# LowLevelAI/GLARE

Measured on AMD Instinct MI355X. Metric: enhanced images/sec (400x600), higher is better.
Workload: dtype fp16; 1 GPU; LOL eval15-shaped 400x600 inference, batch=8 per GPU, full encoder->flow->VQ->decoder->AFT (BASELINE configs[1]); batch_per_gpu=8, global_batch=8, input=3x400x600 (reflect-padded to 420x620), parallelism=dp1, streams_per_gpu=2, exchange=none (1 GPU), ranks_seen=1, weights=random, name-seeded (no checkpoints offline)

## Files before the change

### glare_amd/csrc/attn.hip

```cpp
#include <type_traits>

#include "common.h"

namespace {

constexpr int AT_THREADS = 256;
constexpr int HD = 512;
constexpr int BM = 128;
constexpr int BN = 32;
constexpr int KCH = BN * (HD / 8);
constexpr float RESCALE_THR = 8.0f;
constexpr int ATTN_DMA_PER_GROUP = 2;

__device__ __forceinline__ void dma16a(const void* gsrc, void* lds_wave_base) {
  __builtin_amdgcn_global_load_lds((const __attribute__((address_space(1))) void*)gsrc,
                                   (__attribute__((address_space(3))) void*)lds_wave_base, 16, 0, 0);
}

template <int N, typename F>
__device__ __forceinline__ void static_for(F&& f) {
  if constexpr (N > 0) {
    static_for<N - 1>(f);
    f(std::integral_constant<int, N - 1>{});
  }
}

struct AttnParams {
  const a16_t* q;
  const a16_t* k;
  const a16_t* vt;
  a16_t* o;
  int B, N;
  long long Npad;
  int ldq, ldk, ldo;
  int n_qblocks, n_blocks;
  int key_splits;
  float* part_o;
  float* part_ml;
  float* lse;
  a16_t* o_lo;
};

__global__ __launch_bounds__(AT_THREADS, 1) void attn_fwd_kernel(const AttnParams p) {
  extern __shared__ __attribute__((aligned(16))) char smem[];
  u32x4* lK = reinterpret_cast<u32x4*>(smem);
  u32x4* lV = lK + 2 * KCH;

  int bid = blockIdx.x;
  {
    const int n = p.n_blocks, q = n / 8, r = n % 8, xcd = bid % 8, kk = bid / 8;
    bid = (xcd < r ? xcd * (q + 1) : r * (q + 1) + (xcd - r) * q) + kk;
  }
  const int qb = bid % p.n_qblocks, ksplit = (bid / p.n_qblocks) % p.key_splits, b = bid / (p.n_qblocks * p.key_splits);
  const int tid = threadIdx.x, lane = tid & 63;
  const int wave = __builtin_amdgcn_readfirstlane(tid >> 6);
  const int ql = lane & 31, hi = lane >> 5;
  const int qrow = qb * BM + wave * 32 + ql;
  const bool q_ok = qrow < p.N;

  a16x8 qf[HD / 16];
  {
    const a16_t* qp = p.q + ((size_t)b * p.N + (q_ok ? qrow : 0)) * p.ldq + hi * 8;
#pragma unroll
    for (int ks = 0; ks < HD / 16; ++ks) {
      u32x4 v = *reinterpret_cast<const u32x4*>(qp + ks * 16);
      if (!q_ok) v = u32x4{0u, 0u, 0u, 0u};
      qf[ks] = __builtin_bit_cast(a16x8, v);
    }
  }

  f32x16 o[HD / 32];
#pragma unroll
  for (int i = 0; i < HD / 32; ++i)
#pragma unroll
    for (int r = 0; r < 16; ++r) o[i][r] = 0.f;
  float m_run = -1e30f, l_run = 0.f;

  const int n_tiles = (p.N + BN - 1) / BN;
  const int t_begin = (int)((long long)n_tiles * ksplit / p.key_splits), t_end = (int)((long long)n_tiles * (ksplit + 1) / p.key_splits);
  const a16_t* kbase = p.k + (size_t)b * p.N * p.ldk;
  const a16_t* vbase = p.vt + (size_t)b * HD * p.Npad;

  const unsigned v_lane_off = (unsigned)((lane >> 2) * p.Npad + (((lane & 3) ^ ((lane >> 4) & 3)) * 8)) * 2u;
  const __amdgpu_buffer_rsrc_t krsrc = __builtin_amdgcn_make_buffer_rsrc(
      const_cast<a16_t*>(kbase), 0, (int)((((long long)p.N - 1) * p.ldk + HD) * 2), 0x00020000);
  const __amdgpu_buffer_rsrc_t vrsrc =
      __builtin_amdgcn_make_buffer_rsrc(const_cast<a16_t*>(vbase), 0, (int)((long long)HD * p.Npad * 2), 0x00020000);
  const int lane16 = lane * 16;
  auto issue_piece = [&](auto ic, int tile, int buf) {
    constexpr int i = decltype(ic)::value;
    if constexpr (i < BN / 4) {
      const int r = wave + 4 * i;
      __builtin_amdgcn_raw_ptr_buffer_load_lds(krsrc, (__attribute__((address_space(3))) void*)(lK + buf * KCH + r * 64), 16,
                                               lane16 ^ ((r & 15) * 16), (tile * BN + r) * p.ldk * 2, 0, 0);
    } else {
      constexpr int j = i - BN / 4;
      __builtin_amdgcn_raw_ptr_buffer_load_lds(vrsrc, (__attribute__((address_space(3))) void*)(lV + buf * KCH + (wave + 4 * j) * 64), 16,
                                               v_lane_off, (int)(((long long)(wave + 4 * j) * 16 * p.Npad + (long long)tile * BN) * 2), 0, 0);
    }
  };
  auto issue = [&](int tile, int buf) { static_for<16>([&](auto ic) { issue_piece(ic, tile, buf); }); };

  const int krow = (ql & 0x13) | ((ql & 4) << 1) | ((ql & 8) >> 1);
  const int kswz = krow & 15;

  int kofs[8], vofs[2];
#pragma unroll
  for (int bb = 0; bb < 8; ++bb) kofs[bb] = (krow * 64 + ((2 * bb + hi) ^ kswz)) * 16;
#pragma unroll
  for (int ks = 0; ks < 2; ++ks) vofs[ks] = 2 * KCH * 16 + (ql * 4 + ((2 * ks + hi) ^ ((ql >> 2) & 3))) * 16;

  auto tile_body = [&](auto bufc, int tile) {
    constexpr int BUF = decltype(bufc)::value;
    asm volatile("s_waitcnt vmcnt(0)" ::: "memory");
    __syncthreads();
    const int nxt = min(tile + 1, t_end - 1);
    const char* kb = smem + BUF * KCH * 16;
    const char* vb = smem + BUF * KCH * 16;
    a16x8 fr[3][4];
    auto ldk = [&](auto gc, a16x8(&f)[4]) {
      constexpr int g = decltype(gc)::value;
#pragma unroll
      for (int e = 0; e < 4; ++e) {
        const int ks = 4 * g + e;
        f[e] = *reinterpret_cast<const a16x8*>(kb + kofs[ks & 7] + (ks >> 3) * 256);
      }
    };
    auto ldv = [&](auto gc, a16x8(&f)[4]) {
      constexpr int g = decltype(gc)::value;
#pragma unroll
      for (int e = 0; e < 4; ++e) f[e] = *reinterpret_cast<const a16x8*>(vb + vofs[e & 1] + (2 * g + (e >> 1)) * 2048);
    };

    f32x16 s;
#pragma unroll
    for (int r = 0; r < 16; ++r) s[r] = 0.f;
    ldk(std::integral_constant<int, 0>{}, fr[0]);
    ldk(std::integral_constant<int, 1>{}, fr[1]);
    static_for<8>([&](auto gc) {
      constexpr int g = decltype(gc)::value;
      if constexpr (g + 2 < 8) ldk(std::integral_constant<int, g + 2>{}, fr[(g + 2) % 3]);
      else ldv(std::integral_constant<int, g + 2 - 8>{}, fr[(g + 2) % 3]);
      static_for<ATTN_DMA_PER_GROUP>([&](auto kc) {
        constexpr int piece = g * ATTN_DMA_PER_GROUP + decltype(kc)::value;
        if constexpr (piece < 16) issue_piece(std::integral_constant<int, piece>{}, nxt, BUF ^ 1);
      });
#pragma unroll
      for (int e = 0; e < 4; ++e) s = mfma_a16_32x32x16(fr[g % 3][e], qf[4 * g + e], s, 0, 0, 0);
      __builtin_amdgcn_sched_barrier(0);
    });
    if (tile == n_tiles - 1) {
#pragma unroll
      for (int r = 0; r < 16; ++r) {
        const int kv = tile * BN + 16 * (r >> 3) + 8 * hi + (r & 7);
        if (kv >= p.N) s[r] = -__builtin_inff();
      }
    }
    float mx = s[0];
#pragma unroll
    for (int r = 1; r < 16; ++r) mx = fmaxf(mx, s[r]);
    {
      const auto sw = __builtin_amdgcn_permlane32_swap(__float_as_uint(mx), __float_as_uint(mx), false, false);
      mx = fmaxf(mx, __uint_as_float(hi ? sw[0] : sw[1]));
    }
    if (__any(mx > m_run + RESCALE_THR)) {
      const float m_new = fmaxf(m_run, mx);
      const float alpha = __builtin_amdgcn_exp2f(m_run - m_new);
      l_run *= alpha;
#pragma unroll
      for (int i = 0; i < HD / 32; ++i)
#pragma unroll
        for (int r = 0; r < 16; ++r) {
          float x = o[i][r], tmp;
          asm volatile("v_accvgpr_read_b32 %1, %0\n\tv_mul_f32 %1, %1, %2\n\tv_accvgpr_write_b32 %0, %1"
                       : "+a"(x), "=&v"(tmp)
                       : "v"(alpha));
          o[i][r] = x;
        }
      m_run = m_new;
    }
    float psum = 0.f;
    a16x8 pf[2];
#pragma unroll
    for (int h = 0; h < 2; ++h) {
      u32x4 w;
#pragma unroll
      for (int e = 0; e < 4; ++e) {
        const float p0 = __builtin_amdgcn_exp2f(s[8 * h + 2 * e] - m_run);
        const float p1 = __builtin_amdgcn_exp2f(s[8 * h + 2 * e + 1] - m_run);
        psum += p0 + p1;
        w[e] = pack_a2(p0, p1);
      }
      pf[h] = __builtin_bit_cast(a16x8, w);
    }
    l_run += psum;
    __builtin_amdgcn_sched_barrier(0);
    static_for<8>([&](auto gc) {
      constexpr int g = decltype(gc)::value;
      if constexpr (g + 2 < 8) ldv(std::integral_constant<int, g + 2>{}, fr[(8 + g + 2) % 3]);
      static_for<ATTN_DMA_PER_GROUP>([&](auto kc) {
        constexpr int piece = (8 + g) * ATTN_DMA_PER_GROUP + decltype(kc)::value;
        if constexpr (piece < 16) issue_piece(std::integral_constant<int, piece>{}, nxt, BUF ^ 1);
      });
#pragma unroll
      for (int e = 0; e < 4; ++e)
        o[2 * g + (e >> 1)] = mfma_a16_32x32x16(fr[(8 + g) % 3][e], pf[e & 1], o[2 * g + (e >> 1)], 0, 0, 0);
      __builtin_amdgcn_sched_barrier(0);
    });
  };

  issue(t_begin, 0);
  for (int tile = t_begin; tile < t_end; tile += 2) {
    tile_body(std::integral_constant<int, 0>{}, tile);
    if (tile + 1 < t_end) tile_body(std::integral_constant<int, 1>{}, tile + 1);
  }


  const float l_tot = l_run + __shfl_xor(l_run, 32, 64);
  if (p.key_splits > 1) {
    if (q_ok) {
      const size_t row = ((size_t)b * p.key_splits + ksplit) * p.N + qrow;
      float* po = p.part_o + row * HD;
#pragma unroll
      for (int dt = 0; dt < HD / 32; ++dt)
#pragma unroll
        for (int rq = 0; rq < 4; ++rq) {
          const int d = dt * 32 + 8 * rq + 4 * hi;
          *reinterpret_cast<f32x4*>(po + d) = f32x4{o[dt][4 * rq], o[dt][4 * rq + 1], o[dt][4 * rq + 2], o[dt][4 * rq + 3]};
        }
      if (hi == 0) { p.part_ml[row * 2] = m_run; p.part_ml[row * 2 + 1] = l_tot; }
    }
    return;
  }
  const float inv = 1.0f / l_tot;
  if (p.lse && q_ok && hi == 0) p.lse[(size_t)b * p.N + qrow] = m_run + __builtin_amdgcn_logf(l_tot);
  if (q_ok) {
    a16_t* op = p.o + ((size_t)b * p.N + qrow) * p.ldo;
#pragma unroll
    for (int dt = 0; dt < HD / 32; ++dt)
#pragma unroll
      for (int rq = 0; rq < 4; ++rq) {
        const int d = dt * 32 + 8 * rq + 4 * hi;
        u32x2 w = {pack_a2(o[dt][4 * rq] * inv, o[dt][4 * rq + 1] * inv),
                   pack_a2(o[dt][4 * rq + 2] * inv, o[dt][4 * rq + 3] * inv)};
        *reinterpret_cast<u32x2*>(op + d) = w;
      }
  }
}

typedef __attribute__((ext_vector_type(4))) short s16x4;


__device__ __forceinline__ int kv_swz(int key) { return ((key & 3) << 2) | ((key >> 2) & 3); }

template <int OFF>
__device__ __forceinline__ void tr_read_b64(u32x2& dst, int addr) {
  asm volatile("ds_read_b64_tr_b16 %0, %1 offset:%2" : "=v"(dst) : "v"(addr), "i"(OFF));
}
template <int N>
__device__ __forceinline__ void lgkm_wait8(u32x2 (&f)[8]) {
  asm volatile("s_waitcnt lgkmcnt(%8)"
               : "+v"(f[0]), "+v"(f[1]), "+v"(f[2]), "+v"(f[3]), "+v"(f[4]), "+v"(f[5]), "+v"(f[6]), "+v"(f[7])
               : "i"(N));
}

template <bool PAIR>
__global__ __launch_bounds__(AT_THREADS, 1) void attn_kv_fwd_kernel(const AttnParams p) {
  extern __shared__ __attribute__((aligned(16))) char smem[];
  u32x4* lKV = reinterpret_cast<u32x4*>(smem);

  int bid = blockIdx.x;
  {
    const int n = p.n_blocks, q = n / 8, r = n % 8, xcd = bid % 8, kk = bid / 8;
    bid = (xcd < r ? xcd * (q + 1) : r * (q + 1) + (xcd - r) * q) + kk;
  }
  const int qb = bid % p.n_qblocks, ksplit = (bid / p.n_qblocks) % p.key_splits, b = bid / (p.n_qblocks * p.key_splits);
  const int tid = threadIdx.x, lane = tid & 63;
  const int wave = __builtin_amdgcn_readfirstlane(tid >> 6);
  const int ql = lane & 31, hi = lane >> 5;
  const int qrow = qb * BM + wave * 32 + ql;
  const bool q_ok = qrow < p.N;

  a16x8 qf[HD / 16];
  {
    const a16_t* qp = p.q + ((size_t)b * p.N + (q_ok ? qrow : 0)) * p.ldq + hi * 8;
#pragma unroll
    for (int ks = 0; ks < HD / 16; ++ks) {
      u32x4 v = *reinterpret_cast<const u32x4*>(qp + ks * 16);
      if (!q_ok) v = u32x4{0u, 0u, 0u, 0u};
      qf[ks] = __builtin_bit_cast(a16x8, v);
    }
  }
  f32x16 o[HD / 32];
#pragma unroll
  for (int i = 0; i < HD / 32; ++i)
#pragma unroll
    for (int r = 0; r < 16; ++r) o[i][r] = 0.f;
  float m_run = -1e30f, l_run = 0.f;

  const int n_tiles = (p.N + BN - 1) / BN;
  const int t_begin = (int)((long long)n_tiles * ksplit / p.key_splits), t_end = (int)((long long)n_tiles * (ksplit + 1) / p.key_splits);
  const a16_t* kbase = p.k + (size_t)b * p.N * p.ldk;
  const __amdgpu_buffer_rsrc_t krsrc = __builtin_amdgcn_make_buffer_rsrc(
      const_cast<a16_t*>(kbase), 0, (int)((((long long)p.N - 1) * p.ldk + HD) * 2), 0x00020000);
  const int lane16w = (lane ^ (wave << 2)) * 16;
  auto issue_piece = [&](auto ic, int tile, int buf) {
    constexpr int i = decltype(ic)::value;
    const int r = wave + 4 * i;
    __builtin_amdgcn_raw_ptr_buffer_load_lds(krsrc, (__attribute__((address_space(3))) void*)(lKV + buf * KCH + r * 64), 16,
                                             lane16w ^ ((i & 3) * 16), (tile * BN + r) * p.ldk * 2, 0, 0);
  };

  const int krow = (ql & 0x13) | ((ql & 4) << 1) | ((ql & 8) >> 1);
  const int kf = kv_swz(krow);
  int kofs[8];
#pragma unroll
  for (int bb = 0; bb < 8; ++bb) kofs[bb] = (krow * 64 + ((2 * bb + hi) ^ kf)) * 16;
  int vofs[4][2];
  {
    const int i16 = lane & 15, g4 = (lane >> 4) & 1;
#pragma unroll
    for (int dtl = 0; dtl < 4; ++dtl)
#pragma unroll
      for (int h = 0; h < 2; ++h) {
        const int key = 8 * hi + 4 * h + (i16 >> 2);
        const int chunk = 4 * dtl + 2 * g4 + ((i16 & 3) >> 1);
        vofs[dtl][h] = key * 1024 + ((chunk ^ kv_swz(key)) * 16) + (i16 & 1) * 8;
      }
  }

#define PROF_MARK(i) do {} while (0)
  auto tile_body = [&](auto bufc, int tile) {
    constexpr int BUF = decltype(bufc)::value;
    PROF_MARK(0);
    asm volatile("s_waitcnt vmcnt(0)" ::: "memory");
    __syncthreads();
    PROF_MARK(1);
    const int nxt = min(tile + 1, t_end - 1);
    const char* tb = smem + BUF * KCH * 16;
    a16x8 fr[3][4];
    auto ldk = [&](auto gc, a16x8(&f)[4]) {
      constexpr int g = decltype(gc)::value;
#pragma unroll
      for (int e = 0; e < 4; ++e) {
        const int ks = 4 * g + e;
        f[e] = *reinterpret_cast<const a16x8*>(tb + kofs[ks & 7] + (ks >> 3) * 256);
      }
    };
    auto ldv1 = [&](auto gc, auto ic, u32x2(&f)[8]) {
      constexpr int g = decltype(gc)::value, i = decltype(ic)::value, e = i >> 1;
      constexpr int dt = 2 * g + (e >> 1), ks = e & 1;
      tr_read_b64<BUF * KCH * 16 + ks * 16384 + (dt >> 2) * 256>(f[i], vofs[dt & 3][i & 1]);
    };
    auto ldv = [&](auto gc, u32x2(&f)[8]) {
      static_for<8>([&](auto ic) { ldv1(gc, ic, f); });
    };
    auto wait_v = [&](auto nc, u32x2(&f)[8]) {
      lgkm_wait8<decltype(nc)::value>(f);
    };
    auto vfrag = [&](const u32x2(&f)[8], int e) {
      return __builtin_bit_cast(a16x8, u32x4{f[2 * e][0], f[2 * e][1], f[2 * e + 1][0], f[2 * e + 1][1]});
    };
    u32x2 vf[2][8];

    f32x16 s;
#pragma unroll
    for (int r = 0; r < 16; ++r) s[r] = 0.f;
    ldk(std::integral_constant<int, 0>{}, fr[0]);
    ldk(std::integral_constant<int, 1>{}, fr[1]);
    static_for<8>([&](auto gc) {
      constexpr int g = decltype(gc)::value;
      if constexpr (g + 2 < 8) ldk(std::integral_constant<int, g + 2>{}, fr[(g + 2) % 3]);
      issue_piece(gc, nxt, BUF ^ 1);
#pragma unroll
      for (int e = 0; e < 4; ++e) s = mfma_a16_32x32x16(fr[g % 3][e], qf[4 * g + e], s, 0, 0, 0);
      __builtin_amdgcn_sched_barrier(0);
    });
    PROF_MARK(2);
    ldv(std::integral_constant<int, 0>{}, vf[0]);
    if (tile == n_tiles - 1) {
#pragma unroll
      for (int r = 0; r < 16; ++r) {
        const int kv = tile * BN + 16 * (r >> 3) + 8 * hi + (r & 7);
        if (kv >= p.N) s[r] = -__builtin_inff();
      }
    }
    float mx = s[0];
#pragma unroll
    for (int r = 1; r < 16; ++r) mx = fmaxf(mx, s[r]);
    {
      const auto sw = __builtin_amdgcn_permlane32_swap(__float_as_uint(mx), __float_as_uint(mx), false, false);
      mx = fmaxf(mx, __uint_as_float(hi ? sw[0] : sw[1]));
    }
    if (__any(mx > m_run + RESCALE_THR)) {
      const float m_new = fmaxf(m_run, mx);
      const float alpha = __builtin_amdgcn_exp2f(m_run - m_new);
      l_run *= alpha;
#pragma unroll
      for (int i = 0; i < HD / 32; ++i)
#pragma unroll
        for (int r = 0; r < 16; ++r) {
          float x = o[i][r], tmp;
          asm volatile("v_accvgpr_read_b32 %1, %0\n\tv_mul_f32 %1, %1, %2\n\tv_accvgpr_write_b32 %0, %1"
                       : "+a"(x), "=&v"(tmp)
                       : "v"(alpha));
          o[i][r] = x;
        }
      m_run = m_new;
    }
    float psum = 0.f;
    a16x8 pf[2];
#pragma unroll
    for (int h = 0; h < 2; ++h) {
      u32x4 w;
#pragma unroll
      for (int e = 0; e < 4; ++e) {
        const float p0 = __builtin_amdgcn_exp2f(s[8 * h + 2 * e] - m_run);
        const float p1 = __builtin_amdgcn_exp2f(s[8 * h + 2 * e + 1] - m_run);
        psum += p0 + p1;
        w[e] = pack_a2(p0, p1);
      }
      pf[h] = __builtin_bit_cast(a16x8, w);
    }
    l_run += psum;
    __builtin_amdgcn_sched_barrier(0);
    PROF_MARK(3);
    static_for<8>([&](auto gc) {
      constexpr int g = decltype(gc)::value;
      if constexpr (g + 1 < 8) {
        ldv(std::integral_constant<int, g + 1>{}, vf[(g + 1) & 1]);
        wait_v(std::integral_constant<int, 8>{}, vf[g & 1]);
      } else {
        wait_v(std::integral_constant<int, 0>{}, vf[g & 1]);
      }
#define VF_CUR vf[g & 1]
#pragma unroll
      for (int e = 0; e < 4; ++e)
        o[2 * g + (e >> 1)] = mfma_a16_32x32x16(vfrag(VF_CUR, e), pf[e & 1], o[2 * g + (e >> 1)], 0, 0, 0);
      __builtin_amdgcn_sched_barrier(0);
    });
    PROF_MARK(4);
  };

  static_for<8>([&](auto ic) { issue_piece(ic, t_begin, 0); });
  for (int tile = t_begin; tile < t_end; tile += 2) {
    tile_body(std::integral_constant<int, 0>{}, tile);
    if (tile + 1 < t_end) tile_body(std::integral_constant<int, 1>{}, tile + 1);
  }

  const float l_tot = l_run + __shfl_xor(l_run, 32, 64);
  if (p.key_splits > 1) {
    if (q_ok) {
      const size_t row = ((size_t)b * p.key_splits + ksplit) * p.N + qrow;
      float* po = p.part_o + row * HD;
#pragma unroll
      for (int dt = 0; dt < HD / 32; ++dt)
#pragma unroll
        for (int rq = 0; rq < 4; ++rq) {
          const int d = dt * 32 + 8 * rq + 4 * hi;
          *reinterpret_cast<f32x4*>(po + d) = f32x4{o[dt][4 * rq], o[dt][4 * rq + 1], o[dt][4 * rq + 2], o[dt][4 * rq + 3]};
        }
      if (hi == 0) { p.part_ml[row * 2] = m_run; p.part_ml[row * 2 + 1] = l_tot; }
    }
    return;
  }
  const float inv = 1.0f / l_tot;
  if (q_ok) {
    a16_t* op = p.o + ((size_t)b * p.N + qrow) * p.ldo;
#pragma unroll
    for (int dt = 0; dt < HD / 32; ++dt)
#pragma unroll
      for (int rq = 0; rq < 4; ++rq) {
        const int d = dt * 32 + 8 * rq + 4 * hi;
        u32x2 w = {pack_a2(o[dt][4 * rq] * inv, o[dt][4 * rq + 1] * inv),
                   pack_a2(o[dt][4 * rq + 2] * inv, o[dt][4 * rq + 3] * inv)};
        *reinterpret_cast<u32x2*>(op + d) = w;
        if constexpr (PAIR) {
          const u32x2 l = {pack_a2(o[dt][4 * rq] * inv - alo(w[0]), o[dt][4 * rq + 1] * inv - ahi(w[0])),
                           pack_a2(o[dt][4 * rq + 2] * inv - alo(w[1]), o[dt][4 * rq + 3] * inv - ahi(w[1]))};
          *reinterpret_cast<u32x2*>(p.o_lo + ((size_t)b * p.N + qrow) * p.ldo + d) = l;
        }
      }
  }
}


__global__ __launch_bounds__(256) void attn_combine_kernel(const float* __restrict__ part_o, const float* __restrict__ part_ml,
                                                           a16_t* __restrict__ out, int ldo, int B, int N, int KS,
                                                           float* __restrict__ lse, a16_t* __restrict__ out_lo = nullptr) {
  const long long row = (long long)blockIdx.x * 4 + (threadIdx.x >> 6);
  if (row >= (long long)B * N) return;
  const int lane = threadIdx.x & 63, b = (int)(row / N), q = (int)(row % N);
  float m = -1e30f;
  for (int s = 0; s < KS; ++s) m = fmaxf(m, part_ml[(((size_t)b * KS + s) * N + q) * 2]);
  float acc[8], L = 0.f;
#pragma unroll
  for (int e = 0; e < 8; ++e) acc[e] = 0.f;
  for (int s = 0; s < KS; ++s) {
    const size_t r = ((size_t)b * KS + s) * N + q;
    const float w = __builtin_amdgcn_exp2f(part_ml[r * 2] - m);
    L += w * part_ml[r * 2 + 1];
    const f32x4 v0 = *reinterpret_cast<const f32x4*>(part_o + r * HD + lane * 8);
    const f32x4 v1 = *reinterpret_cast<const f32x4*>(part_o + r * HD + lane * 8 + 4);
#pragma unroll
    for (int e = 0; e < 4; ++e) { acc[e] = fmaf(w, v0[e], acc[e]); acc[4 + e] = fmaf(w, v1[e], acc[4 + e]); }
  }
  const float inv = 1.0f / L;
  if (lse && lane == 0) lse[row] = m + __builtin_amdgcn_logf(L);
  u32x4 o = {pack_a2(acc[0] * inv, acc[1] * inv), pack_a2(acc[2] * inv, acc[3] * inv), pack_a2(acc[4] * inv, acc[5] * inv),
             pack_a2(acc[6] * inv, acc[7] * inv)};
  *reinterpret_cast<u32x4*>(out + (size_t)row * ldo + lane * 8) = o;
  if (out_lo) {
    u32x4 l;
#pragma unroll
    for (int e = 0; e < 4; ++e) l[e] = pack_a2(acc[2 * e] * inv - alo(o[e]), acc[2 * e + 1] * inv - ahi(o[e]));
    *reinterpret_cast<u32x4*>(out_lo + (size_t)row * ldo + lane * 8) = l;
  }
}

}

static int attn_launch(const void* q, int ldq, const void* k, int ldk, const void* v_t, long long v_pitch, void* out, int ldo, int B,
                       int N, int key_splits, void* workspace, size_t workspace_bytes, glare_stream_t stream, float* lse = nullptr);

extern "C" int glare_attention_d512_lse_bf16(const void* q, int ldq, const void* k, int ldk, const void* v_t, long long v_pitch, void* out,
                                             int ldo, float* lse, int B, int N, int key_splits, void* workspace, size_t workspace_bytes,
                                             glare_stream_t stream) {
  if (!lse) return GLARE_ERR_INVALID;
  return attn_launch(q, ldq, k, ldk, v_t, v_pitch, out, ldo, B, N, key_splits, workspace, workspace_bytes, stream, lse);
}

extern "C" size_t glare_attention_d512_splitk_workspace_bytes(int B, int N, int key_splits) {
  if (B <= 0 || N <= 0 || key_splits <= 1) return 0;
  return (size_t)B * key_splits * N * (HD + 2) * sizeof(float);
}

extern "C" int glare_attention_d512_splitk_bf16(const void* q, int ldq, const void* k, int ldk, const void* v_t, long long v_pitch,
                                                void* out, int ldo, int B, int N, int key_splits, void* workspace,
                                                size_t workspace_bytes, glare_stream_t stream) {
  return attn_launch(q, ldq, k, ldk, v_t, v_pitch, out, ldo, B, N, key_splits, workspace, workspace_bytes, stream);
}

extern "C" int glare_attention_kv512_bf16(const void* q, int ldq, const void* kv, int ldkv, void* out, int ldo, int B, int N,
                                          int key_splits, void* workspace, size_t workspace_bytes, glare_stream_t stream) {
  return glare_attention_kv512_pair_bf16(q, ldq, kv, ldkv, out, nullptr, ldo, B, N, key_splits, workspace, workspace_bytes, stream);
}

extern "C" int glare_attention_kv512_pair_bf16(const void* q, int ldq, const void* kv, int ldkv, void* out, void* out_lo, int ldo, int B,
                                               int N, int key_splits, void* workspace, size_t workspace_bytes, glare_stream_t stream) {
  if (!q || !kv || !out || B <= 0 || N <= 0 || key_splits < 1) return GLARE_ERR_INVALID;
  if (key_splits > (N + BN - 1) / BN) return GLARE_ERR_INVALID;
  if (((long long)N * ldkv + HD) * 2 >= 0x7ff00000LL) return GLARE_ERR_UNSUPPORTED;
  if (key_splits > 1 &&
      ((ldo % 8) || !workspace || workspace_bytes < glare_attention_d512_splitk_workspace_bytes(B, N, key_splits)))
    return GLARE_ERR_WORKSPACE;
  if ((ldq % 8) || (ldkv % 8) || (ldo % 4) || ldq < HD || ldkv < HD || ldo < HD) return GLARE_ERR_UNSUPPORTED;
  AttnParams p;
  p.q = (const a16_t*)q; p.k = (const a16_t*)kv; p.vt = nullptr; p.o = (a16_t*)out; p.o_lo = (a16_t*)out_lo;
  p.B = B; p.N = N; p.Npad = 0; p.ldq = ldq; p.ldk = ldkv; p.ldo = ldo; p.lse = nullptr;
  p.n_qblocks = (N + BM - 1) / BM;
  p.key_splits = key_splits;
  p.part_o = static_cast<float*>(workspace);
  p.part_ml = p.part_o ? p.part_o + (size_t)B * key_splits * N * HD : nullptr;
  const long long nb = (long long)B * p.n_qblocks * key_splits;
  if (nb > 0x7fffffffLL) return GLARE_ERR_INVALID;
  p.n_blocks = (int)nb;
  const size_t lds = (size_t)2 * KCH * 16;
  auto kern = (out_lo && key_splits == 1) ? attn_kv_fwd_kernel<true> : attn_kv_fwd_kernel<false>;
  if (hipFuncSetAttribute((const void*)kern, hipFuncAttributeMaxDynamicSharedMemorySize, (int)lds) != hipSuccess)
    return GLARE_ERR_LAUNCH;
  hipLaunchKernelGGL(kern, dim3(p.n_blocks), dim3(AT_THREADS), lds, (hipStream_t)stream, p);
  if (key_splits > 1)
    hipLaunchKernelGGL(attn_combine_kernel, dim3((unsigned)(((long long)B * N + 3) / 4)), dim3(256), 0, (hipStream_t)stream, p.part_o,
                       p.part_ml, p.o, ldo, B, N, key_splits, (float*)nullptr, p.o_lo);
  return glare_launch_status();
}

extern "C" int glare_attention_d512_bf16(const void* q, int ldq, const void* k, int ldk, const void* v_t,
                                         long long v_pitch, void* out, int ldo, int B, int N, glare_stream_t stream) {
  return attn_launch(q, ldq, k, ldk, v_t, v_pitch, out, ldo, B, N, 1, nullptr, 0, stream);
}

static int attn_launch(const void* q, int ldq, const void* k, int ldk, const void* v_t, long long v_pitch, void* out, int ldo, int B,
                       int N, int key_splits, void* workspace, size_t workspace_bytes, glare_stream_t stream, float* lse) {
  if (!q || !k || !v_t || !out || B <= 0 || N <= 0 || key_splits < 1) return GLARE_ERR_INVALID;
  
  if (key_splits > (N + BN - 1) / BN) return GLARE_ERR_INVALID;
  if (((long long)N * ldk + HD) * 2 >= 0x7ff00000LL || (long long)HD * v_pitch * 2 >= 0x7ff00000LL) return GLARE_ERR_UNSUPPORTED;
  if (key_splits > 1) {

    if ((ldo % 8) || !workspace || workspace_bytes < glare_attention_d512_splitk_workspace_bytes(B, N, key_splits)) return GLARE_ERR_WORKSPACE;
  }
  if ((ldq % 8) || (ldk % 8) || (ldo % 4) || (v_pitch % 8) || ldq < HD || ldk < HD || ldo < HD) return GLARE_ERR_UNSUPPORTED;
  if (v_pitch < (long long)((N + BN - 1) / BN) * BN) return GLARE_ERR_INVALID;
  AttnParams p;
  p.q = (const a16_t*)q; p.k = (const a16_t*)k; p.vt = (const a16_t*)v_t; p.o = (a16_t*)out; p.o_lo = nullptr;
  p.B = B; p.N = N; p.Npad = v_pitch; p.ldq = ldq; p.ldk = ldk; p.ldo = ldo; p.lse = lse;
  p.n_qblocks = (N + BM - 1) / BM;
  p.key_splits = key_splits;
  p.part_o = static_cast<float*>(workspace);
  p.part_ml = p.part_o ? p.part_o + (size_t)B * key_splits * N * HD : nullptr;
  const long long nb = (long long)B * p.n_qblocks * key_splits;
  if (nb > 0x7fffffffLL) return GLARE_ERR_INVALID;
  p.n_blocks = (int)nb;
  const size_t lds = (size_t)4 * KCH * 16;
  if (hipFuncSetAttribute((const void*)attn_fwd_kernel, hipFuncAttributeMaxDynamicSharedMemorySize, (int)lds) != hipSuccess)
    return GLARE_ERR_LAUNCH;
  hipLaunchKernelGGL(attn_fwd_kernel, dim3(p.n_blocks), dim3(AT_THREADS), lds, (hipStream_t)stream, p);
  if (key_splits > 1)
    hipLaunchKernelGGL(attn_combine_kernel, dim3((unsigned)(((long long)B * N + 3) / 4)), dim3(256), 0, (hipStream_t)stream, p.part_o,
                       p.part_ml, p.o, ldo, B, N, key_splits, lse);
  return glare_launch_status();
}
```

Measured before the change: 64.06 images/sec.

## Make KV-attention DMA placement configurable and interleave V loads with PV MFMAs

Adds a compile-time placement table that decides where in the tile body each of the 8 next-tile DMA pieces is issued: during the QK MFMA groups, inside the softmax steps, or during the PV groups. The default keeps all pieces in the QK phase. The PV loop now interleaves per-fragment V LDS reads with the MFMAs using finer-grained lgkmcnt waits, so transposed reads overlap matrix math instead of being issued in bulk. Optional s_memtime stamp instrumentation is added behind a macro. The finer waits and sched barriers may limit compiler scheduling freedom.

```diff
diff --git a/glare_amd/csrc/attn.hip b/glare_amd/csrc/attn.hip
--- a/glare_amd/csrc/attn.hip
+++ b/glare_amd/csrc/attn.hip
@@ -11,6 +11,32 @@
 constexpr int KCH = BN * (HD / 8);
 constexpr float RESCALE_THR = 8.0f;
 constexpr int ATTN_DMA_PER_GROUP = 2;
+
+#ifndef ATTN_KV_PLACE
+#define ATTN_KV_PLACE 1,1,1,1,1,1,1,1,0,0,0,0,0,0,0,0,0
+#endif
+#ifndef ATTN_KV_PV_INTERLEAVE
+#define ATTN_KV_PV_INTERLEAVE 1
+#endif
+constexpr bool KV_PV_INTERLEAVE = ATTN_KV_PV_INTERLEAVE;
+constexpr int KV_SLOTS = 17, KV_SLOT_SOFTMAX = 8, KV_SOFTMAX_STEPS = 8;
+constexpr int KV_PLACE[KV_SLOTS] = {ATTN_KV_PLACE};
+constexpr int kv_place_first(int slot) {
+  int n = 0;
+  for (int s = 0; s < slot; ++s) n += KV_PLACE[s];
+  return n;
+}
+static_assert(kv_place_first(KV_SLOTS) == BN / 4, "ATTN_KV_PLACE must place exactly the 8 pieces of a tile");
+constexpr int kv_softmax_pieces_before(int step) {
+  const int n = KV_PLACE[KV_SLOT_SOFTMAX];
+  int c = 0;
+  for (int k = 0; k < n; ++k) c += (k * KV_SOFTMAX_STEPS / (n > 0 ? n : 1) < step);
+  return c;
+}
+constexpr int kv_softmax_valu_per_piece() {
+  const int n = KV_PLACE[KV_SLOT_SOFTMAX];
+  return 56 / (n > 0 ? n : 1);
+}
 
 __device__ __forceinline__ void dma16a(const void* gsrc, void* lds_wave_base) {
   __builtin_amdgcn_global_load_lds((const __attribute__((address_space(1))) void*)gsrc,
@@ -39,7 +65,19 @@
   float* part_ml;
   float* lse;
   a16_t* o_lo;
+#ifdef GLARE_ATTN_STAMPS
+  unsigned long long* stamps;
+#endif
 };
+
+#ifdef GLARE_ATTN_STAMPS
+constexpr int ATTN_STAMPS = 6;
+__device__ __forceinline__ unsigned long long attn_stamp() {
+  unsigned long long t;
+  asm volatile("s_memtime %0\n\ts_waitcnt lgkmcnt(0)" : "=s"(t) : : "memory");
+  return t;
+}
+#endif
 
 __global__ __launch_bounds__(AT_THREADS, 1) void attn_fwd_kernel(const AttnParams p) {
   extern __shared__ __attribute__((aligned(16))) char smem[];
@@ -264,6 +302,11 @@
                : "i"(N));
 }
 
+template <int N>
+__device__ __forceinline__ void lgkm_wait2(u32x2& a, u32x2& b) {
+  asm volatile("s_waitcnt lgkmcnt(%2)" : "+v"(a), "+v"(b) : "i"(N));
+}
+
 template <bool PAIR>
 __global__ __launch_bounds__(AT_THREADS, 1) void attn_kv_fwd_kernel(const AttnParams p) {
   extern __shared__ __attribute__((aligned(16))) char smem[];
@@ -329,7 +372,31 @@
       }
   }
 
+  auto issue_slot = [&](auto sc, int tile, int buf) {
+    constexpr int slot = decltype(sc)::value, first = kv_place_first(slot);
+    static_for<KV_PLACE[slot]>([&](auto kc) { issue_piece(std::integral_constant<int, first + decltype(kc)::value>{}, tile, buf); });
+  };
+  auto issue_softmax_step = [&](auto stepc, int tile, int buf) {
+    constexpr int step = decltype(stepc)::value;
+    constexpr int lo = kv_softmax_pieces_before(step), n = kv_softmax_pieces_before(step + 1) - lo;
+    static_for<n>([&](auto kc) {
+      issue_piece(std::integral_constant<int, kv_place_first(KV_SLOT_SOFTMAX) + lo + decltype(kc)::value>{}, tile, buf);
+    });
+  };
+
+#ifdef GLARE_ATTN_STAMPS
+  unsigned long long st[ATTN_STAMPS] = {0, 0, 0, 0, 0, 0};
+  const int stamp_tile = t_begin + (t_end - t_begin) / 2;
+#define PROF_MARK(i)                                                        \
+  do {                                                                      \
+    __builtin_amdgcn_sched_barrier(0);                                      \
+    if (tile == stamp_tile) st[i] = attn_stamp();                           \
+    if ((i) == 0 && tile == stamp_tile + 1) st[ATTN_STAMPS - 1] = attn_stamp(); \
+    __builtin_amdgcn_sched_barrier(0);                                      \
+  } while (0)
+#else
 #define PROF_MARK(i) do {} while (0)
+#endif
   auto tile_body = [&](auto bufc, int tile) {
     constexpr int BUF = decltype(bufc)::value;
     PROF_MARK(0);
@@ -371,7 +438,7 @@
     static_for<8>([&](auto gc) {
       constexpr int g = decltype(gc)::value;
       if constexpr (g + 2 < 8) ldk(std::integral_constant<int, g + 2>{}, fr[(g + 2) % 3]);
-      issue_piece(gc, nxt, BUF ^ 1);
+      issue_slot(gc, nxt, BUF ^ 1);
 #pragma unroll
       for (int e = 0; e < 4; ++e) s = mfma_a16_32x32x16(fr[g % 3][e], qf[4 * g + e], s, 0, 0, 0);
       __builtin_amdgcn_sched_barrier(0);
@@ -410,34 +477,53 @@
     }
     float psum = 0.f;
     a16x8 pf[2];
-#pragma unroll
-    for (int h = 0; h < 2; ++h) {
-      u32x4 w;
-#pragma unroll
-      for (int e = 0; e < 4; ++e) {
-        const float p0 = __builtin_amdgcn_exp2f(s[8 * h + 2 * e] - m_run);
-        const float p1 = __builtin_amdgcn_exp2f(s[8 * h + 2 * e + 1] - m_run);
-        psum += p0 + p1;
-        w[e] = pack_a2(p0, p1);
-      }
-      pf[h] = __builtin_bit_cast(a16x8, w);
-    }
+    u32x4 pw[2];
+    static_for<KV_SOFTMAX_STEPS>([&](auto stepc) {
+      constexpr int step = decltype(stepc)::value, h = step >> 2, e = step & 3;
+      const float p0 = __builtin_amdgcn_exp2f(s[8 * h + 2 * e] - m_run);
+      const float p1 = __builtin_amdgcn_exp2f(s[8 * h + 2 * e + 1] - m_run);
+      psum += p0 + p1;
+      pw[h][e] = pack_a2(p0, p1);
+      issue_softmax_step(stepc, nxt, BUF ^ 1);
+    });
+    pf[0] = __builtin_bit_cast(a16x8, pw[0]);
+    pf[1] = __builtin_bit_cast(a16x8, pw[1]);
     l_run += psum;
+    {
+      static_for<KV_PLACE[KV_SLOT_SOFTMAX]>([&](auto) {
+        __builtin_amdgcn_sched_group_barrier(0x002, kv_softmax_valu_per_piece(), 0);
+        __builtin_amdgcn_sched_group_barrier(0x010, 1, 0);
+      });
+    }
     __builtin_amdgcn_sched_barrier(0);
     PROF_MARK(3);
     static_for<8>([&](auto gc) {
       constexpr int g = decltype(gc)::value;
-      if constexpr (g + 1 < 8) {
-        ldv(std::integral_constant<int, g + 1>{}, vf[(g + 1) & 1]);
-        wait_v(std::integral_constant<int, 8>{}, vf[g & 1]);
+      issue_slot(std::integral_constant<int, KV_SLOT_SOFTMAX + 1 + g>{}, nxt, BUF ^ 1);
+#define VF_CUR vf[g & 1]
+      if constexpr (KV_PV_INTERLEAVE) {
+        static_for<4>([&](auto ec) {
+          constexpr int e = decltype(ec)::value;
+          lgkm_wait2<(g + 1 < 8) ? 6 : 6 - 2 * e>(VF_CUR[2 * e], VF_CUR[2 * e + 1]);
+          o[2 * g + (e >> 1)] = mfma_a16_32x32x16(vfrag(VF_CUR, e), pf[e & 1], o[2 * g + (e >> 1)], 0, 0, 0);
+          if constexpr (g + 1 < 8) {
+            ldv1(std::integral_constant<int, g + 1>{}, std::integral_constant<int, 2 * e>{}, vf[(g + 1) & 1]);
+            ldv1(std::integral_constant<int, g + 1>{}, std::integral_constant<int, 2 * e + 1>{}, vf[(g + 1) & 1]);
+          }
+          __builtin_amdgcn_sched_barrier(0);
+        });
       } else {
-        wait_v(std::integral_constant<int, 0>{}, vf[g & 1]);
-      }
-#define VF_CUR vf[g & 1]
-#pragma unroll
-      for (int e = 0; e < 4; ++e)
-        o[2 * g + (e >> 1)] = mfma_a16_32x32x16(vfrag(VF_CUR, e), pf[e & 1], o[2 * g + (e >> 1)], 0, 0, 0);
-      __builtin_amdgcn_sched_barrier(0);
+        if constexpr (g + 1 < 8) {
+          ldv(std::integral_constant<int, g + 1>{}, vf[(g + 1) & 1]);
+          wait_v(std::integral_constant<int, 8>{}, vf[g & 1]);
+        } else {
+          wait_v(std::integral_constant<int, 0>{}, vf[g & 1]);
+        }
+#pragma unroll
+        for (int e = 0; e < 4; ++e)
+          o[2 * g + (e >> 1)] = mfma_a16_32x32x16(vfrag(VF_CUR, e), pf[e & 1], o[2 * g + (e >> 1)], 0, 0, 0);
+        __builtin_amdgcn_sched_barrier(0);
+      }
     });
     PROF_MARK(4);
   };
@@ -447,6 +533,13 @@
     tile_body(std::integral_constant<int, 0>{}, tile);
     if (tile + 1 < t_end) tile_body(std::integral_constant<int, 1>{}, tile + 1);
   }
+#ifdef GLARE_ATTN_STAMPS
+  if (p.stamps && lane == 0) {
+    unsigned long long* sp = p.stamps + ((size_t)blockIdx.x * (AT_THREADS / 64) + wave) * ATTN_STAMPS;
+#pragma unroll
+    for (int i = 0; i < ATTN_STAMPS; ++i) sp[i] = st[i];
+  }
+#endif
 
   const float l_tot = l_run + __shfl_xor(l_run, 32, 64);
   if (p.key_splits > 1) {
@@ -565,6 +658,13 @@
   const long long nb = (long long)B * p.n_qblocks * key_splits;
   if (nb > 0x7fffffffLL) return GLARE_ERR_INVALID;
   p.n_blocks = (int)nb;
+#ifdef GLARE_ATTN_STAMPS
+  p.stamps = nullptr;
+  if (key_splits == 1 && workspace) {
+    if (workspace_bytes < (size_t)p.n_blocks * (AT_THREADS / 64) * ATTN_STAMPS * sizeof(unsigned long long)) return GLARE_ERR_WORKSPACE;
+    p.stamps = static_cast<unsigned long long*>(workspace);
+  }
+#endif
   const size_t lds = (size_t)2 * KCH * 16;
   auto kern = (out_lo && key_splits == 1) ? attn_kv_fwd_kernel<true> : attn_kv_fwd_kernel<false>;
   if (hipFuncSetAttribute((const void*)kern, hipFuncAttributeMaxDynamicSharedMemorySize, (int)lds) != hipSuccess)
```

Result: faster. 65.22 images/sec, median of 6 (+1.8%).
